# EspressoSystems/Push-CDN

Measured on NVIDIA H100. Metric: broadcast fan-out egress GB/s (1 KiB x 2^20 subscribers per GPU, 1 topic); msgs/s and % of HBM peak alongside, higher is better.
Workload: dtype u8

## Files before the change

### push-cdn_b200/csrc/engine.cu

```cuda
#include "engine_internal.h"

namespace pcdn_detail {
thread_local std::string g_err;
int fail(int code, const std::string& msg) { g_err = msg; return code; }
}

namespace {

int flush_journal(pcdn_engine* e) {
  HostTables& t = *e->tables;
  if (!e->has_device) { t.clear_dirty(); return 0; }
  const Geometry& g = e->geo;
  bool any = !t.dirty_sub.empty() || !t.dirty_brk.empty() || !t.dirty_owner.empty() || !t.dirty_slots.empty() ||
             !t.dirty_keys.empty();
  if (!any) return 0;
  const uint32_t Ws = e->shard_W(), W = g.W;
  const bool full_keys = t.dirty_keys.size() > (size_t)g.max_keys / 16 + 64;
  const bool full_sub = t.dirty_sub.size() > t.sub.size() / 16 + 64;
  const bool full_slots = t.dirty_slots.size() > t.cuckoo.size() / 16 + 64;
  e->h_slot.clear(); e->h_kslot.clear(); e->h_kbytes.clear();
  if (!full_slots) for (uint32_t i : t.dirty_slots) e->h_slot.push_back(UpdSlot{i, t.cuckoo[i]});
  if (!full_keys) for (uint32_t k : t.dirty_keys) {
    e->h_kslot.push_back(k);
    size_t at = e->h_kbytes.size();
// ... 148 lines not shown
  if (sh.dev.pool && !fused) s.spans_mapped = false;
  s.w.spans = s.spans_mapped ? s.d_spans_map : s.d_spans_dev;
  s.w.overflow = s.spans_mapped ? s.d_ovf_map : s.d_ovf_dev;
  const bool zero_in_kernel = fused && !devparse && !retry;
  const bool zero_in_match = !fused && !devparse && !retry && !has_direct && s.in.n_bcast > 0;
  if (s.timed) CUDA_TRY(cudaEventRecord(s.ev[0], st));
  if (retry) {
    launch_pool_retry_begin(sh.dev, s.w, st);
  } else {
    if (!zero_in_kernel && !zero_in_match) launch_batch_begin(sh.dev, s.w, s.in, has_direct, st);
    if (devparse) launch_parse(sh.dev, s.w, s.in, st);
    if (has_direct && !fused) launch_direct(sh.dev, s.w, s.in, n_direct, st);
  }
  if (s.timed) CUDA_TRY(cudaEventRecord(s.ev[1], st));
  if (fused) {
    launch_ctrl_small(sh.dev, s.w, s.in, has_direct, hs.targeted, zero_in_kernel, s.d_stats_pub, retry, st);
    if (s.timed) { CUDA_TRY(cudaEventRecord(s.ev[2], st)); CUDA_TRY(cudaEventRecord(s.ev[3], st)); }
  } else {
    if (!retry) launch_match(sh.dev, s.w, s.in, zero_in_match ? s.w.stats : nullptr, hs.targeted, st);
    if (s.timed) CUDA_TRY(cudaEventRecord(s.ev[2], st));
    if (!retry) launch_plan(sh.dev, s.w, s.in, st);
    launch_offsets(sh.dev, s.w, s.in, has_direct, sh.n_sms, st);
    if (s.timed) CUDA_TRY(cudaEventRecord(s.ev[3], st));
  }
  if (!s.spans_mapped) {
    CUDA_TRY(cudaEventRecord(s.ev_ctrl, st));
    CUDA_TRY(cudaStreamWaitEvent(cs, s.ev_ctrl, 0));
    CUDA_TRY(cudaMemcpyAsync(s.h_early, s.w.stats, sizeof(BatchStats), cudaMemcpyDeviceToHost, cs));
    CUDA_TRY(cudaEventRecord(s.ev_early, cs));
    if (ps != st) CUDA_TRY(cudaStreamWaitEvent(ps, s.ev_ctrl, 0));
  }
  if (s.timed) CUDA_TRY(cudaEventRecord(s.ev[4], ps));
  uint32_t pack_variant = e->cfg.pack_variant;
  if (!((pack_variant >> 8) & 15u)) pack_variant |= (fat_overlap ? 3u : 4u) << 8;
  const bool has_ref = e->cfg.ref_min_bytes && (hs.device_input || hs.max_raw_len >= e->cfg.ref_min_bytes);
  const bool published = launch_pack(sh.dev, s.w, s.in, n_direct, pack_variant, sh.n_sms, has_ref, fused ? nullptr : s.d_stats_pub, ps);
  if (s.timed) CUDA_TRY(cudaEventRecord(s.ev[5], ps));
// ... 577 lines not shown
    DEV_ALLOC(d.pool_state, 1);
    launch_pool_init(d, sh.stream);
  }
  CUDA_TRY(cudaMemsetAsync(d.sub, 0, (size_t)g.T * Ws * 4, sh.stream));
  CUDA_TRY(cudaMemsetAsync(d.brk, 0, (size_t)Ws * 4, sh.stream));
  CUDA_TRY(cudaMemsetAsync(d.owner_conn, 0xFF, (size_t)g.max_owners * 4, sh.stream));
  CUDA_TRY(cudaMemsetAsync(d.cuckoo, 0, (size_t)g.nbuckets * 4 * sizeof(CuckooEntry), sh.stream));
  CUDA_TRY(cudaMemsetAsync(d.keys, 0, (size_t)g.max_keys * g.key_stride, sh.stream));
  CUDA_TRY(cudaMemsetAsync(d.ptail, 0, (size_t)Ns * 4, sh.stream));
  CUDA_TRY(cudaMemsetAsync(d.used, 0, (size_t)Ns * 4, sh.stream));

  const uint32_t M = c.max_batch_msgs, MB = c.max_batch_bcast;
  const size_t cap_fat = (size_t)c.max_batch_deliveries;
  const size_t cap_thin = std::min<size_t>(c.max_batch_deliveries, (size_t)M * (kFatMin - 1));
  sh.slots.resize(c.batch_slots);
  for (ShardSlot& s : sh.slots) {
    DEV_ALLOC(s.d_arena, e->arena_cap);
    Work& w = s.w;
    DEV_ALLOC(w.B, (size_t)MB * Ws);
    DEV_ALLOC(w.wpre, (size_t)MB * Ws);
    DEV_ALLOC(w.cnt, (size_t)MB * d.nblk);
    DEV_ALLOC(w.base, (size_t)MB * d.nblk);
    DEV_ALLOC(w.done, MB);
    CUDA_TRY(cudaMemsetAsync(w.done, 0, (size_t)MB * 4, sh.stream));
    DEV_ALLOC(w.D, M);
    DEV_ALLOC(w.dconn, M);
    DEV_ALLOC(w.eb_fat, (size_t)M + 1);
    DEV_ALLOC(w.eb_thin, (size_t)M + 1);
    DEV_ALLOC(w.tbase, (size_t)M + 1);
    DEV_ALLOC(w.scan_tmp, 4 * ((size_t)M / 256 + 2));
    DEV_ALLOC(w.cls, M);
    DEV_ALLOC(w.cm_rank, (size_t)M + 1);
    DEV_ALLOC(w.cm_list, MB);
    DEV_ALLOC(w.jidx, M);
    DEV_ALLOC(w.efat, cap_fat);
    DEV_ALLOC(w.ecm, cap_fat);
    DEV_ALLOC(w.cmrun, std::min<size_t>(((size_t)MB + kCmGroup - 1) / kCmGroup * Ns, 2 * cap_fat + Ns));
    DEV_ALLOC(w.ethin, cap_thin);
    w.cap_fat = (uint32_t)std::min<size_t>(cap_fat, 0xFFFFFFFFu);
    w.cap_thin = (uint32_t)std::min<size_t>(cap_thin, 0xFFFFFFFFu);
    DEV_ALLOC(w.dcount, (size_t)Ns + 2);
    DEV_ALLOC(w.dloc, (size_t)Ns + 2);
    DEV_ALLOC(w.dtile, (size_t)Ns / 1024 + 3);
    DEV_ALLOC(w.dlist, M);
    DEV_ALLOC(w.hot_list, (size_t)M / kHotMin + 2);
    DEV_ALLOC(w.hot_bitmap, (size_t)kHotCtas * ((size_t)M / 32 + 1));
    DEV_ALLOC(w.scan_done, 1);
    CUDA_TRY(cudaMemsetAsync(w.scan_done, 0, 4, sh.stream));
    DEV_ALLOC(w.edir, M);
    DEV_ALLOC(w.dstart, (size_t)Ns + 1);
    DEV_ALLOC(w.dend, (size_t)Ns + 1);
    DEV_ALLOC(w.dstamp, (size_t)Ns + 1);
    CUDA_TRY(cudaMemsetAsync(w.dstamp, 0, ((size_t)Ns + 1) * 4, sh.stream));
    w.stamp = 0;
    DEV_ALLOC(w.batch_units, Ns);
    if (d.pool) {
      DEV_ALLOC(w.cbase, Ns);
      DEV_ALLOC(w.lb_state, (size_t)Ns / 256 + 1);
      DEV_ALLOC(w.lb_tot, (size_t)Ns / 256 + 1);
      CUDA_TRY(cudaMemsetAsync(w.lb_state, 0, ((size_t)Ns / 256 + 1) * 8, sh.stream));
    }
    w.pool_unblock = 0;
    const size_t span_entries = (size_t)2 * Ns * (d.span_runs ? 3 : 2) / 2;
    DEV_ALLOC(s.d_spans_dev, span_entries);
    DEV_ALLOC(s.d_ovf_dev, Ns);
    if (sh.direct_publish) {
      PIN_ALLOC_MAPPED(s.h_spans, s.d_spans_map, span_entries);
      PIN_ALLOC_MAPPED(s.h_overflow, s.d_ovf_map, (size_t)Ns);
    } else {
      PIN_ALLOC(s.h_spans, span_entries);
// ... 781 lines not shown
int pcdn_release_batch(pcdn_engine* e, uint64_t batch_id) {
  GUARD_BEGIN
  LOCK;
  const int si = find_slot_index(e, batch_id);
  if (si < 0) return fail(PCDN_ENOENT, "unknown batch id");
  if (e->inflight.empty() || e->inflight.front() != batch_id)
    return fail(PCDN_EINVAL, "batches must be released oldest first");
  Slot& s = e->slots[si];
  for (Shard& sh : e->shards) {
    DeviceGuard dg(sh.device);
    ShardSlot& ss = sh.slots[si];
    const bool payload_copy = s.device_input && e->delivers_by_ref();
    if (!ss.polled && (!s.device_input || payload_copy))
      CUDA_TRY(cudaEventSynchronize((e->sharded && !payload_copy) ? ss.ev_ingest : ss.ev_done));
    CUDA_TRY(cudaStreamWaitEvent(sh.stream, ss.ev_done, 0));
    launch_release(sh.dev, ss.w.batch_units, ss.w.stats, sh.stream);
    CUDA_TRY(cudaGetLastError());
  }
  e->inflight.erase(e->inflight.begin());
  s.state = SLOT_FREE;
  e->inflight_bytes -= std::min(e->inflight_bytes, s.ingress_bytes);
  s.ingress_bytes = 0;
  e->stats.released_batches++;
  {
    const double ms = std::chrono::duration<double, std::milli>(std::chrono::steady_clock::now() - s.t_launch).count();
    e->stats.latency_ms_sum += ms;
    const uint64_t us = (uint64_t)(ms * 1000.0);
    int bucket = 0;
    while (bucket < 15 && us >= (16ull << bucket)) bucket++;
    e->stats.latency_hist_us[bucket]++;
  }
// ... 115 lines not shown
```

### push-cdn_b200/csrc/engine_internal.h

```cpp
#pragma once
#include <cuda_runtime.h>

#include <algorithm>
#include <chrono>
#include <cstdio>
#include <cstring>
#include <memory>
#include <mutex>
#include <new>
#include <string>
#include <thread>
#include <vector>

#include "frame_parse.h"
#include "host_state.h"
#include "kernels.cuh"
#include "nccl_dl.h"
#include "pcdn_fanout.h"

using namespace pcdn;

namespace pcdn_detail {

int fail(int code, const std::string& msg);
// ... 69 lines not shown
struct Shard {
  int device = 0;
  uint32_t gindex = 0;
  int n_sms = 132;
  bool direct_publish = false;
  uint8_t* h_rings = nullptr;
  cudaStream_t stream = nullptr, pack_stream = nullptr, copy_stream = nullptr, ingest_stream = nullptr;
  bool own_stream = false;
  DevState dev{};
  std::vector<ShardSlot> slots;
  uint8_t* jstage_h = nullptr; uint8_t* jstage_d = nullptr; size_t jstage_cap = 0;
  cudaEvent_t ev_journal = nullptr; bool ev_journal_pending = false;
  std::vector<Upd32> h_u32;
  NcclComm comm = nullptr;
  int nccl_ranks = 0;
  int prev_slot[2] = {-1, -1};
  bool fat_only = false;
  cudaEvent_t ev_submit = nullptr;
  std::vector<void*> dev_allocs, pin_allocs;
};

struct Slot {
  int state = SLOT_FREE;
  uint64_t batch_id = 0;
  bool device_input = false;
  uint8_t* h_arena = nullptr;
  size_t arena_used = 0;
  std::vector<uint8_t> kind, flags;
  std::vector<uint32_t> slot_off16, raw_len, aux_off, aux_len, bcast_index;
  std::vector<uint16_t> topics;
// ... 119 lines not shown
```

### push-cdn_b200/csrc/kernels.cu

```cuda
#include "kernels.cuh"

#include <atomic>

#include "frame_parse_core.h"

namespace pcdn {

std::atomic<unsigned long long> g_kernel_launches{0};
#define PCDN_COUNT_LAUNCH (void)g_kernel_launches.fetch_add(1, std::memory_order_relaxed)

unsigned long long kernel_launches() { return g_kernel_launches.load(std::memory_order_relaxed); }
void count_kernel_launch() { PCDN_COUNT_LAUNCH; }

__device__ __forceinline__ uint32_t lane_id() { return threadIdx.x & 31; }

__device__ __forceinline__ uint32_t warp_incl_scan(uint32_t v) {
  const uint32_t lane = lane_id();
#pragma unroll
  for (int o = 1; o < 32; o <<= 1) {
    uint32_t n = __shfl_up_sync(0xffffffffu, v, o);
    if (lane >= (uint32_t)o) v += n;
  }
  return v;
}
// ... 288 lines not shown

void launch_batch_begin(const DevState&, const Work& w, const BatchIn&, bool, cudaStream_t st) {
  cudaMemsetAsync(w.stats, 0, sizeof(BatchStats), st);
}

void launch_direct(const DevState& s, const Work& w, const BatchIn& b, uint32_t n_direct, cudaStream_t st) {
  const uint32_t n = b.n_msgs;
  const uint32_t nseg = s.N + 1, ntiles = (nseg + 1023) / 1024;
  cudaMemsetAsync(w.dcount, 0, (size_t)(s.N + 2) * 4, st);
  PCDN_COUNT_LAUNCH, k_direct_lookup<<<(n * 8 + 255) / 256, 256, 0, st>>>(s, b, w);
  PCDN_COUNT_LAUNCH, k_dscan<<<ntiles, 256, 0, st>>>(w, nseg, ntiles);
  PCDN_COUNT_LAUNCH, k_dfill<<<(n + 255) / 256, 256, 0, st>>>(b, w);
  if (n_direct > kHotMin) PCDN_COUNT_LAUNCH, k_dsort_hot<<<kHotCtas, 256, 0, st>>>(b, w, (n + 31) / 32);
}


__device__ __forceinline__ bool msg_topic(const DevState& s, const BatchIn& b, uint32_t fl, uint32_t toff, uint32_t i, uint32_t* t) {
  if (fl & MSGF_TOPICS_U8) {
    const uint8_t* tb = b.arena + toff;
    if ((fl & MSGF_PRUNE) && !topic_kept(tb, i, s.n_valid_topics)) return false;
    *t = tb[i];
  } else {
    *t = b.topics[toff + i];
  }
  return *t < s.T;
}

__device__ uint32_t event_bit(const DevState& s, const BatchIn& b, uint32_t m, uint32_t wd, uint32_t k, uint32_t e0, uint32_t e1) {
  const uint32_t fl = b.flags[m], toff = b.aux_off[m], tn = b.aux_len[m];
  for (uint32_t i = 0; i < tn; i++) {
// ... 53 lines not shown
    for (uint32_t i = 0; i < tn; i++) {
      if ((fl & MSGF_PRUNE) && !topic_kept(tb, i, s.n_valid_topics)) continue;
      const uint32_t t = tb[i];
      if (t < s.T) word |= s.sub[(size_t)t * s.W + wd];
    }
  } else {
    for (uint32_t i = 0; i < tn; i++) {
      const uint32_t t = b.topics[toff + i];
      if (t < s.T) word |= s.sub[(size_t)t * s.W + wd];
    }
  }
  if (b.n_events) apply_events<1>(s, b, m, wd, &word);
  if (fl & MSGF_USERS_ONLY) word &= ~s.brk[wd];
  return word;
}
template <bool EVENTS, bool TARGET>
__global__ void __launch_bounds__(256) k_match(DevState s, BatchIn b, Work w, BatchStats* zero) {
  if (zero && blockIdx.x == 0 && blockIdx.y == 0 && threadIdx.x < sizeof(BatchStats) / 4) reinterpret_cast<uint32_t*>(zero)[threadIdx.x] = 0;
  const uint32_t j = blockIdx.y, lane = lane_id();
  const uint32_t blk = blockIdx.x * 8 + (threadIdx.x >> 5);
  if (blk >= s.nblk) return;
  const uint32_t m = b.bcast_index[j];
  const uint32_t w0 = blk * kBlockWords + lane * 8;
  const uint32_t toff = b.aux_off[m], tn = b.aux_len[m], fl = b.flags[m];
  uint4 lo = make_uint4(0, 0, 0, 0), hi = make_uint4(0, 0, 0, 0);
  auto or_row = [&](uint32_t t) {
    if (t >= s.T) return;
    const uint4* row = reinterpret_cast<const uint4*>(s.sub + (size_t)t * s.W + w0);
    const uint4 a = row[0], c = row[1];
    lo.x |= a.x; lo.y |= a.y; lo.z |= a.z; lo.w |= a.w;
    hi.x |= c.x; hi.y |= c.y; hi.z |= c.z; hi.w |= c.w;
  };
// ... 20 lines not shown
  if (TARGET && (fl & MSGF_TARGET)) {
    if (toff == kConnNone) {
      const uint4* br = reinterpret_cast<const uint4*>(s.brk + w0);
      lo = br[0]; hi = br[1];
    } else {
      const uint32_t local = toff - s.conn_base, bit = 1u << (local & 31u);
      const uint32_t q = local < s.N ? (local >> 5) - w0 : 8u;
      lo = make_uint4(q == 0 ? bit : 0u, q == 1 ? bit : 0u, q == 2 ? bit : 0u, q == 3 ? bit : 0u);
      hi = make_uint4(q == 4 ? bit : 0u, q == 5 ? bit : 0u, q == 6 ? bit : 0u, q == 7 ? bit : 0u);
    }
  }
  const uint32_t p0 = __popc(lo.x), p1 = p0 + __popc(lo.y), p2 = p1 + __popc(lo.z), p3 = p2 + __popc(lo.w);
  const uint32_t p4 = p3 + __popc(hi.x), p5 = p4 + __popc(hi.y), p6 = p5 + __popc(hi.z), p7 = p6 + __popc(hi.w);
  const uint32_t incl = warp_incl_scan(p7), ex = incl - p7;
  uint32_t last = 0;
  if (lane == 31) {
    w.cnt[(size_t)j * s.nblk + blk] = incl;
    __threadfence();
    last = atomicAdd(&w.done[j], 1u) == s.nblk - 1 ? 1u : 0u;
  }
  uint4* Bo = reinterpret_cast<uint4*>(w.B + (size_t)j * s.W + w0);
  Bo[0] = lo; Bo[1] = hi;
  uint4 pre;
  pre.x = ex | ((ex + p0) << 16); pre.y = (ex + p1) | ((ex + p2) << 16);
  pre.z = (ex + p3) | ((ex + p4) << 16); pre.w = (ex + p5) | ((ex + p6) << 16);
  *reinterpret_cast<uint4*>(w.wpre + (size_t)j * s.W + w0) = pre;
  if (__shfl_sync(0xffffffffu, last, 31)) {
    __threadfence();
    uint32_t carry = 0;
    for (uint32_t bb = 0; bb < s.nblk; bb += 32) {
      const uint32_t i = bb + lane;
      const uint32_t v = i < s.nblk ? __ldcg(w.cnt + (size_t)j * s.nblk + i) : 0;
      const uint32_t in = warp_incl_scan(v);
      if (i < s.nblk) w.base[(size_t)j * s.nblk + i] = carry + in - v;
      carry += __shfl_sync(0xffffffffu, in, 31);
    }
    if (lane == 0) { w.D[m] = carry; w.jidx[m] = j; w.done[j] = 0; }
  }
}
void launch_match(const DevState& s, const Work& w, const BatchIn& b, BatchStats* zero, bool targeted, cudaStream_t st) {
  if (!b.n_bcast) return;
  dim3 grid((s.nblk + 7) / 8, b.n_bcast);
  if (targeted) {
    if (b.n_events) PCDN_COUNT_LAUNCH, k_match<true, true><<<grid, 256, 0, st>>>(s, b, w, zero);
    else PCDN_COUNT_LAUNCH, k_match<false, true><<<grid, 256, 0, st>>>(s, b, w, zero);
  } else {
    if (b.n_events) PCDN_COUNT_LAUNCH, k_match<true, false><<<grid, 256, 0, st>>>(s, b, w, zero);
    else PCDN_COUNT_LAUNCH, k_match<false, false><<<grid, 256, 0, st>>>(s, b, w, zero);
  }
}

__device__ __forceinline__ uint32_t frame_vec_bytes(uint32_t raw_len) { return (4u + raw_len + 15u) & ~15u; }
__device__ __forceinline__ uint32_t frame_units(uint32_t raw_len) { return (4u + raw_len + kUnit - 1u) / kUnit; }
__device__ __forceinline__ bool by_ref(const DevState& s, uint32_t raw_len) { return raw_len >= s.ref_min; }
__device__ __forceinline__ uint32_t rec_units(const DevState& s, uint32_t raw_len) {
  return by_ref(s, raw_len) ? 1u : frame_units(raw_len);
}
__device__ __forceinline__ uint32_t tile_recipients(uint32_t frame_bytes) {
  const uint32_t chunk = min(frame_bytes, kChunkBytes);
  return max(32u, min(kTileRecipients, kFatTileBytes / chunk));
}

__device__ __forceinline__ void plan_classify(const DevState& s, const BatchIn& b, uint32_t m, uint32_t d, uint32_t* cls_out,
                                              uint32_t* tiles_out) {
  uint32_t cls = CLS_THIN, tiles = 0;
  if (d >= kFatMin) {
    const uint32_t len = b.raw_len[m];
    const bool ref = by_ref(s, len);
    const bool dense = !ref && ((uint64_t)d << kCmDenseShift) >= s.N && b.kind[m] == 4;
    if (dense && frame_units(len) * kUnit <= kCmMaxBytes) {
      cls = CLS_CM;
    } else {
      cls = CLS_FAT;
      const uint32_t nch = (frame_vec_bytes(len) + kChunkBytes - 1) / kChunkBytes;
      const uint32_t tr = tile_recipients(frame_vec_bytes(len));
      tiles = ref ? 0u : nch * ((d + tr - 1) / tr);
    }
  }
  *cls_out = cls; *tiles_out = tiles;
}

__global__ void __launch_bounds__(256) k_plan_a(DevState s, BatchIn b, Work w, uint32_t nblk) {
  __shared__ uint32_t sm[9];
  const uint32_t m = blockIdx.x * 256 + threadIdx.x;
  const bool valid = m < b.n_msgs;
  const uint32_t d = valid ? w.D[m] : 0;
  uint32_t cls, tiles;
  plan_classify(s, b, m, d, &cls, &tiles);
  uint32_t tot;
  uint32_t e0 = block256_excl_scan(cls != CLS_THIN ? d : 0, &tot, sm);
  if (threadIdx.x == 0) w.scan_tmp[blockIdx.x] = tot;
  uint32_t e1 = block256_excl_scan(cls == CLS_THIN ? d : 0, &tot, sm);
  if (threadIdx.x == 0) w.scan_tmp[nblk + blockIdx.x] = tot;
  uint32_t e2 = block256_excl_scan(tiles, &tot, sm);
  if (threadIdx.x == 0) w.scan_tmp[2 * nblk + blockIdx.x] = tot;
  uint32_t e3 = block256_excl_scan(cls == CLS_CM ? 1u : 0u, &tot, sm);
  if (threadIdx.x == 0) w.scan_tmp[3 * nblk + blockIdx.x] = tot;
  if (valid) { w.eb_fat[m] = e0; w.eb_thin[m] = e1; w.tbase[m] = e2; w.cm_rank[m] = e3; w.cls[m] = (uint8_t)cls; }
  if (gridDim.x == 1) {
    if (valid && cls == CLS_CM) w.cm_list[e3] = m;
    if (threadIdx.x == 0) {
      const uint32_t t0 = w.scan_tmp[0], t1 = w.scan_tmp[1], t2 = w.scan_tmp[2], t3 = w.scan_tmp[3];
      w.stats->n_fat_entries = t0; w.stats->n_thin_entries = t1; w.stats->n_fat_tiles = t2; w.stats->tile_cursor = 0;
      w.stats->n_cm = t3; w.stats->cm_cursor = 0;
      if (t0 > w.cap_fat || t1 > w.cap_thin) w.stats->status = 1;
      const uint32_t n = b.n_msgs;
      w.eb_fat[n] = t0; w.eb_thin[n] = t1; w.tbase[n] = t2; w.cm_rank[n] = t3;
    }
  }
}
__global__ void __launch_bounds__(256) k_plan_b(Work w, uint32_t nblk) {
  __shared__ uint32_t sm[9];
  const uint32_t q = blockIdx.x;
  uint32_t* t = w.scan_tmp + (size_t)q * nblk;
  uint32_t carry = 0;
  for (uint32_t bb = 0; bb < nblk; bb += 256) {
    const uint32_t i = bb + threadIdx.x;
    const uint32_t v = i < nblk ? t[i] : 0;
    uint32_t tot, ex = block256_excl_scan(v, &tot, sm);
    if (i < nblk) t[i] = ex + carry;
    carry += tot;
  }
  if (threadIdx.x == 0) {
    if (q == 0) { w.stats->n_fat_entries = carry; if (carry > w.cap_fat) w.stats->status = 1; }
// ... 7 lines not shown
  if (m < b.n_msgs) {
    w.eb_fat[m] += w.scan_tmp[blockIdx.x];
    w.eb_thin[m] += w.scan_tmp[nblk + blockIdx.x];
    w.tbase[m] += w.scan_tmp[2 * nblk + blockIdx.x];
    const uint32_t r = w.cm_rank[m] + w.scan_tmp[3 * nblk + blockIdx.x];
    w.cm_rank[m] = r;
    if (w.cls[m] == CLS_CM) w.cm_list[r] = m;
  } else if (m == b.n_msgs) {
    w.eb_fat[m] = w.stats->n_fat_entries;
    w.eb_thin[m] = w.stats->n_thin_entries;
    w.tbase[m] = w.stats->n_fat_tiles;
    w.cm_rank[m] = w.stats->n_cm;
  }
}
void launch_plan(const DevState& s, const Work& w, const BatchIn& b, cudaStream_t st) {
  if (b.n_bcast == 0) return;
  const uint32_t nblk = (b.n_msgs + 255) / 256;
  PCDN_COUNT_LAUNCH, k_plan_a<<<nblk, 256, 0, st>>>(s, b, w, nblk);
  if (nblk == 1) return;
  PCDN_COUNT_LAUNCH, k_plan_b<<<4, 256, 0, st>>>(w, nblk);
  PCDN_COUNT_LAUNCH, k_plan_c<<<(b.n_msgs + 1 + 255) / 256, 256, 0, st>>>(b, w, nblk);
}

struct ConnCursor {
  uint32_t pt, us, bu;
  uint32_t s1_off, s1_units, s1_rec, s2_units, s2_rec;
  uint32_t ovf, in2;
  uint32_t bytes;
};
__device__ __forceinline__ uint32_t alloc_record(ConnCursor& k, uint32_t u, uint32_t R, uint32_t raw_len) {
  if (k.ovf) return kOffInvalid;
  const bool wrap = k.pt + u > R;
  const uint32_t pad = wrap ? R - k.pt : 0, at = wrap ? 0 : k.pt;
  if (u > R || k.us + pad + u > R) { k.ovf = 1; return kOffInvalid; }
// ... 50 lines not shown
    if ((unsigned long long)p->head + total <= s.pool_units) ok = true;
    else if (total <= p->tail && p->used) { skip = s.pool_units - p->head; base = 0; ok = true; }
    else ok = false;
    if (p->used && p->head == p->tail) ok = false;
  } else {
    ok = p->head + total <= p->tail;
  }
  if (!ok) { bs->status = 2; p->blocked = 1; return; }
  p->head = base + total;
  p->used += total + skip;
  bs->pool_base = base; bs->pool_units = total; bs->pool_skip = skip;
}

template <bool HAS_DIRECT, int NT, bool SPARSE_BOUNDS, bool LOOKBACK>
__device__ __forceinline__ void offsets_body(const DevState& s, const BatchIn& b, const Work& w, uint32_t max_conns,
                                             uint32_t c, uint32_t vb, uint32_t nvb) {
  constexpr int NW = NT / 32;
  __shared__ uint32_t sm[NW + 1];
  __shared__ unsigned long long red[2][NW];
  __shared__ uint32_t span_base;
  if (w.stats->status) return;
  const uint32_t wd = c >> 5, lane = c & 31, lt = (1u << lane) - 1u;
  const uint32_t R = s.pool ? 0x7FFFFFFFu : s.ring_units;
  ConnCursor k;
  k.pt = s.pool ? 0u : s.ptail[c]; k.us = s.pool ? 0u : s.used[c]; k.bu = 0;
  k.s1_off = 0; k.s1_units = 0; k.s1_rec = 0; k.s2_units = 0; k.s2_rec = 0; k.ovf = 0; k.in2 = 0; k.bytes = 0;
  uint32_t dp = 0, de = 0;
  if (HAS_DIRECT) {
    if (SPARSE_BOUNDS) {
      if (w.dstamp[c] == w.stamp) { dp = w.dstart[c]; de = w.dend[c]; }
    } else {
      dp = dseg_start(w, c); de = dseg_start(w, c + 1);
      if (de - dp >= 2 && de - dp <= kHotMin) {
        for (uint32_t i = dp + 1; i < de; i++) {
          const uint32_t x = w.dlist[i];
          uint32_t j = i;
          while (j > dp && w.dlist[j - 1] > x) { w.dlist[j] = w.dlist[j - 1]; j--; }
          w.dlist[j] = x;
        }
      }
// ... 140 lines not shown
      uint32_t at = span_base + ex;
      if (k.s1_rec) runs[at++] = SpanRun{s.conn_base + c, run_len, s.pool ? k.s1_off : k.s1_off * kUnit, k.s1_units * kUnit, k.s1_rec, s.pool ? k.s1_units : 0u};
      if (k.s2_rec) runs[at] = SpanRun{s.conn_base + c, 1, 0, k.s2_units * kUnit, k.s2_rec, 0};
    }
  } else if (nsp) {
    uint32_t at = span_base + ex;
    if (k.s1_rec) w.spans[at++] = Span{s.conn_base + c, s.pool ? k.s1_off : k.s1_off * kUnit, k.s1_units * kUnit, k.s1_rec};
    if (k.s2_rec) w.spans[at] = Span{s.conn_base + c, 0, k.s2_units * kUnit, k.s2_rec};
  }
  if (k.ovf) {
    uint32_t i = atomicAdd(&w.stats->n_overflow, 1u);
    if (i < max_conns) w.overflow[i] = s.conn_base + c;
  }
}
template <bool HAS_DIRECT>
__global__ void __launch_bounds__(256) k_offsets(DevState s, BatchIn b, Work w, uint32_t max_conns) {
  offsets_body<HAS_DIRECT, 256, false, false>(s, b, w, max_conns, blockIdx.x * 256 + threadIdx.x, blockIdx.x, gridDim.x);
}
__global__ void __launch_bounds__(1024) k_pool_finish(DevState s, Work w, uint32_t nblk) {
  extern __shared__ uint32_t tb[];
  __shared__ uint32_t sm[33];
  __shared__ unsigned long long total_s;
  if (w.stats->status) return;
  unsigned long long carry = 0;
  for (uint32_t b0 = 0; b0 < nblk; b0 += 1024) {
    const uint32_t i = b0 + threadIdx.x;
    const uint32_t v = i < nblk ? w.lb_tot[i] : 0;
    uint32_t tot, ex = cta_excl_scan<32>(v, &tot, sm);
    const unsigned long long at = carry + ex;
    if (i < nblk) tb[i] = at > 0xFFFFFFFFull ? 0xFFFFFFFFu : (uint32_t)at;
    carry += tot;
  }
  if (threadIdx.x == 0) total_s = carry;
  __syncthreads();
  if (blockIdx.x == 0 && threadIdx.x == 0) pool_allocate(s, w, total_s);
  const uint32_t gt = blockIdx.x * 1024 + threadIdx.x, gn = gridDim.x * 1024;
  for (uint32_t c = gt; c < s.N; c += gn) w.cbase[c] += tb[c >> 8];
  if (s.span_runs) {
    SpanRun* r = reinterpret_cast<SpanRun*>(w.spans);
    const uint32_t n = w.stats->n_runs;
    for (uint32_t i = gt; i < n; i += gn) r[i].ring_off += tb[(r[i].conn0 - s.conn_base) >> 8];
  } else {
    const uint32_t n = w.stats->n_spans;
    for (uint32_t i = gt; i < n; i += gn) w.spans[i].ring_off += tb[(w.spans[i].conn - s.conn_base) >> 8];
  }
}

void launch_offsets(const DevState& s, const Work& w, const BatchIn& b, bool has_direct, int n_sms, cudaStream_t st) {
  if (has_direct) PCDN_COUNT_LAUNCH, k_offsets<true><<<s.N / 256, 256, 0, st>>>(s, b, w, s.N);
  else PCDN_COUNT_LAUNCH, k_offsets<false><<<s.N / 256, 256, 0, st>>>(s, b, w, s.N);
  if (s.pool) {
    const uint32_t nblk = s.N / 256;
    if (nblk * 4 > 48u * 1024) cudaFuncSetAttribute(k_pool_finish, cudaFuncAttributeMaxDynamicSharedMemorySize, (int)(nblk * 4));
    PCDN_COUNT_LAUNCH, k_pool_finish<<<std::min<uint32_t>((uint32_t)n_sms, (s.N + 8191) / 8192), 1024, nblk * 4, st>>>(s, w, nblk);
  }
}

__device__ __forceinline__ void cluster_sync_all() {
  asm volatile("barrier.cluster.arrive.release.aligned;\n\tbarrier.cluster.wait.acquire.aligned;" ::: "memory");
}
template <bool HAS_DIRECT, bool TARGET>
__global__ void __cluster_dims__(8, 1, 1) __launch_bounds__(1024, 1)
k_ctrl_small(DevState s, BatchIn b, Work w, int zero_stats, BatchStats* publish, int offsets_only) {
  __shared__ uint32_t sm[33];
  __shared__ uint32_t gbase[5];
  const uint32_t tid = threadIdx.x, rank = blockIdx.x;
  if (zero_stats && rank == 0 && tid < sizeof(BatchStats) / 4) reinterpret_cast<uint32_t*>(w.stats)[tid] = 0;

  if (HAS_DIRECT && rank == 0 && !offsets_only) {
    __shared__ uint32_t skey_s[kSmallCtrlMsgs], sorted_s[kSmallCtrlMsgs];
    __syncthreads();
    for (uint32_t g0 = 0; g0 < b.n_msgs * 8; g0 += 1024) direct_lookup_body<false>(s, b, w, g0 + tid);
    __syncthreads();
    const uint32_t n = b.n_msgs;
    if (tid < n) { const uint32_t t = w.dconn[tid]; skey_s[tid] = t == kConnNone ? s.N : t; }
    __syncthreads();
    if (tid < n) {
      const uint32_t key = skey_s[tid];
// ... 60 lines not shown
    if (valid) {
      w.eb_fat[m] = e0; w.eb_thin[m] = e1; w.tbase[m] = e2; w.cm_rank[m] = e3; w.cls[m] = (uint8_t)cls;
      if (cls == CLS_CM) w.cm_list[e3] = m;
    }
    if (tid == 0) {
      w.stats->n_fat_entries = t0; w.stats->n_thin_entries = t1; w.stats->n_fat_tiles = t2; w.stats->tile_cursor = 0;
      w.stats->n_cm = t3; w.stats->cm_cursor = 0;
      if (t0 > w.cap_fat || t1 > w.cap_thin) w.stats->status = 1;
      const uint32_t n = b.n_msgs;
      w.eb_fat[n] = t0; w.eb_thin[n] = t1; w.tbase[n] = t2; w.cm_rank[n] = t3;
    }
  }
  cluster_sync_all();

  for (uint32_t c0 = 0; c0 < s.N; c0 += 8192)
    offsets_body<HAS_DIRECT, 1024, true, true>(s, b, w, s.N, c0 + rank * 1024 + tid, c0 / 1024 + rank, s.N / 1024);

  if (publish) {
    cluster_sync_all();
    if (rank == 0 && tid < sizeof(BatchStats) / 4)
      reinterpret_cast<uint32_t*>(publish)[tid] = __ldcg(reinterpret_cast<const uint32_t*>(w.stats) + tid);
  }
}
void launch_ctrl_small(const DevState& s, const Work& w, const BatchIn& b, bool has_direct, bool targeted, bool zero_stats,
                       BatchStats* publish, bool offsets_only, cudaStream_t st) {
  const int z = zero_stats ? 1 : 0, oo = offsets_only ? 1 : 0;
  if (targeted) {
    if (has_direct) PCDN_COUNT_LAUNCH, k_ctrl_small<true, true><<<8, 1024, 0, st>>>(s, b, w, z, publish, oo);
    else PCDN_COUNT_LAUNCH, k_ctrl_small<false, true><<<8, 1024, 0, st>>>(s, b, w, z, publish, oo);
  } else {
    if (has_direct) PCDN_COUNT_LAUNCH, k_ctrl_small<true, false><<<8, 1024, 0, st>>>(s, b, w, z, publish, oo);
    else PCDN_COUNT_LAUNCH, k_ctrl_small<false, false><<<8, 1024, 0, st>>>(s, b, w, z, publish, oo);
  }
}

__global__ void k_pool_retry_begin(BatchStats* bs) {
  bs->status = 0;
  bs->n_deliveries = 0; bs->bytes_out = 0;
  bs->n_spans = 0; bs->n_runs = 0; bs->n_overflow = 0;
  bs->tile_cursor = 0; bs->cm_cursor = 0; bs->ctas_done = 0;
}
void launch_pool_retry_begin(const DevState& s, const Work& w, cudaStream_t st) {
  cudaMemsetAsync(w.lb_state, 0, ((size_t)s.N / 256 + 1) * 8, st);
  PCDN_COUNT_LAUNCH, k_pool_retry_begin<<<1, 1, 0, st>>>(w.stats);
}

__device__ __forceinline__ uint8_t* conn_out(const DevState& s, const Work& w, uint32_t conn, uint32_t pool_base) {
// ... 304 lines not shown
  }
  BatchStats* copy_publish = has_ref ? nullptr : publish;
  const bool direct_separate = n_direct >= kThinSeparateMin;
  const uint32_t ctas_per_sm = ((pack_variant >> 8) & 15u) ? ((pack_variant >> 8) & 15u) : 3;
  const uint32_t grid = (uint32_t)n_sms * ctas_per_sm;
  const int do_direct = (n_direct && !direct_separate) ? 1 : 0;
  if (b.n_bcast || do_direct)
    PCDN_COUNT_LAUNCH, k_pack<<<grid, 256, 0, st>>>(s, b, w, do_direct, direct_separate ? nullptr : copy_publish);
  const uint32_t dctas = ((pack_variant >> 12) & 15u) ? ((pack_variant >> 12) & 15u) : 8u;
  if (direct_separate) PCDN_COUNT_LAUNCH, k_pack_direct<<<(uint32_t)n_sms * dctas, 256, 0, st>>>(s, b, w, copy_publish);
  const bool launched = direct_separate || b.n_bcast || do_direct;
  if (has_ref && launched) PCDN_COUNT_LAUNCH, k_pack_ref<<<ref_ctas, 256, 0, st>>>(s, b, w, n_direct ? 1 : 0, publish);
  return launched;
}

__global__ void __launch_bounds__(256) k_release(DevState s, const uint32_t* __restrict__ batch_units,
                                                 const BatchStats* __restrict__ stats) {
  if (stats->status) return;
  const uint32_t i = blockIdx.x * blockDim.x + threadIdx.x;
  if (i * 4 < s.N) {
    const uint4 u = reinterpret_cast<const uint4*>(batch_units)[i];
    if (u.x | u.y | u.z | u.w) {
      uint4* p = reinterpret_cast<uint4*>(s.used) + i;
      uint4 v = *p;
      v.x -= u.x; v.y -= u.y; v.z -= u.z; v.w -= u.w;
      *p = v;
    }
  }
}
__global__ void k_pool_release(PoolState* p, const BatchStats* __restrict__ stats) {
  if (stats->status) return;
  p->used -= stats->pool_units + stats->pool_skip;
  p->tail = stats->pool_base + stats->pool_units;
  if (p->used == 0) { p->head = 0; p->tail = 0; }
}
__global__ void k_pool_init(PoolState* p) { p->head = 0; p->tail = 0; p->used = 0; p->blocked = 0; }
void launch_pool_init(const DevState& s, cudaStream_t st) {
  if (s.pool) PCDN_COUNT_LAUNCH, k_pool_init<<<1, 1, 0, st>>>(s.pool_state);
}
void launch_release(const DevState& s, const uint32_t* batch_units, const BatchStats* stats, cudaStream_t st) {
  if (s.pool) { PCDN_COUNT_LAUNCH, k_pool_release<<<1, 1, 0, st>>>(s.pool_state, stats); return; }
  PCDN_COUNT_LAUNCH, k_release<<<(s.N / 4 + 255) / 256, 256, 0, st>>>(s, batch_units, stats);
}

}
```

### push-cdn_b200/csrc/kernels.cuh

```cuda
#pragma once
#include <cuda_runtime.h>
#include <stdint.h>

#include "hash.h"

namespace pcdn {

constexpr uint32_t kUnit = 32;
constexpr uint32_t kOffInvalid = 0xFFFFFFFFu;
constexpr uint32_t kCmBroken = 0xFFFFFFF0u;
constexpr uint32_t kConnNone = 0xFFFFFFFFu;
constexpr uint32_t kFatMin = 32;
constexpr uint32_t kChunkBytes = 16384;
constexpr uint32_t kTileRecipients = 1024;
constexpr uint32_t kFatTileBytes = 131072;
constexpr uint32_t kBlockWords = 256;
constexpr uint32_t kCmGroup = 8;
constexpr uint32_t kCmMaxBytes = 4096;
constexpr uint32_t kSmallCtrlConns = 65536;
constexpr uint32_t kSmallCtrlMsgs = 256;
constexpr uint32_t kSmallCtrlItems = 256;
constexpr uint32_t kThinSeparateMin = 2048;
constexpr uint32_t kHotMin = 32;
constexpr uint32_t kHotCtas = 32;
// ... 117 lines not shown
  uint32_t* dend;
  uint32_t* dstamp;
  uint32_t stamp;
  uint32_t* cbase;
  unsigned long long* lb_state;
  uint32_t* lb_tot;
  uint32_t pool_unblock;
  unsigned long long batch_id;
  uint32_t* batch_units;
  Span* spans;
  uint32_t* overflow;
  int8_t* msg_status;
  BatchStats* stats;
};

struct Upd32 { uint32_t arr, idx, val; };
struct UpdSlot { uint32_t slot; CuckooEntry e; };

void launch_apply_updates(const DevState& s, const Upd32* u32, uint32_t n32, const UpdSlot* us,
                          uint32_t nslot, const uint32_t* key_slots, const uint8_t* key_bytes,
                          uint32_t nkeys, cudaStream_t st);
void launch_batch_begin(const DevState& s, const Work& w, const BatchIn& b, bool has_direct, cudaStream_t st);
void launch_parse(const DevState& s, const Work& w, const BatchIn& b, cudaStream_t st);
void launch_direct(const DevState& s, const Work& w, const BatchIn& b, uint32_t n_direct, cudaStream_t st);
void launch_match(const DevState& s, const Work& w, const BatchIn& b, BatchStats* zero, bool targeted, cudaStream_t st);
void launch_plan(const DevState& s, const Work& w, const BatchIn& b, cudaStream_t st);
void launch_offsets(const DevState& s, const Work& w, const BatchIn& b, bool has_direct, int n_sms, cudaStream_t st);
void launch_ctrl_small(const DevState& s, const Work& w, const BatchIn& b, bool has_direct, bool targeted, bool zero_stats,
                       BatchStats* publish, bool offsets_only, cudaStream_t st);
void launch_pool_retry_begin(const DevState& s, const Work& w, cudaStream_t st);
bool launch_pack(const DevState& s, const Work& w, const BatchIn& b, uint32_t n_direct, uint32_t pack_variant, int n_sms,
                 bool has_ref, BatchStats* publish, cudaStream_t st);
void launch_release(const DevState& s, const uint32_t* batch_units, const BatchStats* stats, cudaStream_t st);
void launch_pool_init(const DevState& s, cudaStream_t st);
unsigned long long kernel_launches();
void count_kernel_launch();

}
```

Measured before the change: 3034.

## Defer ring releases into offsets kernel and fold small-batch planning into match

Ring-unit releases for completed batches are no longer a separate kernel. A bitmask of pending slots is recorded, and the next offsets or ctrl kernel subtracts those slots' per-connection units from used before computing offsets. Separately, for batches of up to 256 messages, the last match block to finish (found via an atomic counter) does the plan scan inside k_match with warp scans, so k_plan_a is not launched. This cuts kernel launches per batch, at the cost of shared unit buffers per slot, extra loads in offsets, and subtler ordering invariants around status and error paths.

```diff
diff --git a/push-cdn_b200/csrc/engine.cu b/push-cdn_b200/csrc/engine.cu
--- a/push-cdn_b200/csrc/engine.cu
+++ b/push-cdn_b200/csrc/engine.cu
@@ -186,13 +186,15 @@
   }
   if (s.timed) CUDA_TRY(cudaEventRecord(s.ev[1], st));
   if (fused) {
-    launch_ctrl_small(sh.dev, s.w, s.in, has_direct, hs.targeted, zero_in_kernel, s.d_stats_pub, retry, st);
+    launch_ctrl_small(sh.dev, s.w, s.in, has_direct, hs.targeted, zero_in_kernel, s.d_stats_pub, retry, sh.pending_release, st);
+    sh.pending_release.mask = 0;
     if (s.timed) { CUDA_TRY(cudaEventRecord(s.ev[2], st)); CUDA_TRY(cudaEventRecord(s.ev[3], st)); }
   } else {
     if (!retry) launch_match(sh.dev, s.w, s.in, zero_in_match ? s.w.stats : nullptr, hs.targeted, st);
     if (s.timed) CUDA_TRY(cudaEventRecord(s.ev[2], st));
     if (!retry) launch_plan(sh.dev, s.w, s.in, st);
-    launch_offsets(sh.dev, s.w, s.in, has_direct, sh.n_sms, st);
+    launch_offsets(sh.dev, s.w, s.in, has_direct, sh.n_sms, sh.pending_release, st);
+    sh.pending_release.mask = 0;
     if (s.timed) CUDA_TRY(cudaEventRecord(s.ev[3], st));
   }
   if (!s.spans_mapped) {
@@ -800,6 +802,9 @@
   const size_t cap_fat = (size_t)c.max_batch_deliveries;
   const size_t cap_thin = std::min<size_t>(c.max_batch_deliveries, (size_t)M * (kFatMin - 1));
   sh.slots.resize(c.batch_slots);
+  uint32_t* units = nullptr;
+  DEV_ALLOC(units, (size_t)c.batch_slots * Ns);
+  sh.pending_release = PendingRelease{units, 0};
   for (ShardSlot& s : sh.slots) {
     DEV_ALLOC(s.d_arena, e->arena_cap);
     Work& w = s.w;
@@ -807,8 +812,8 @@
     DEV_ALLOC(w.wpre, (size_t)MB * Ws);
     DEV_ALLOC(w.cnt, (size_t)MB * d.nblk);
     DEV_ALLOC(w.base, (size_t)MB * d.nblk);
-    DEV_ALLOC(w.done, MB);
-    CUDA_TRY(cudaMemsetAsync(w.done, 0, (size_t)MB * 4, sh.stream));
+    DEV_ALLOC(w.done, (size_t)MB + 1);
+    CUDA_TRY(cudaMemsetAsync(w.done, 0, ((size_t)MB + 1) * 4, sh.stream));
     DEV_ALLOC(w.D, M);
     DEV_ALLOC(w.dconn, M);
     DEV_ALLOC(w.eb_fat, (size_t)M + 1);
@@ -839,7 +844,7 @@
     DEV_ALLOC(w.dstamp, (size_t)Ns + 1);
     CUDA_TRY(cudaMemsetAsync(w.dstamp, 0, ((size_t)Ns + 1) * 4, sh.stream));
     w.stamp = 0;
-    DEV_ALLOC(w.batch_units, Ns);
+    w.batch_units = units + (size_t)(&s - sh.slots.data()) * Ns;
     if (d.pool) {
       DEV_ALLOC(w.cbase, Ns);
       DEV_ALLOC(w.lb_state, (size_t)Ns / 256 + 1);
@@ -1651,7 +1656,8 @@
     if (!ss.polled && (!s.device_input || payload_copy))
       CUDA_TRY(cudaEventSynchronize((e->sharded && !payload_copy) ? ss.ev_ingest : ss.ev_done));
     CUDA_TRY(cudaStreamWaitEvent(sh.stream, ss.ev_done, 0));
-    launch_release(sh.dev, ss.w.batch_units, ss.w.stats, sh.stream);
+    if (!sh.dev.pool && (uint32_t)si < kMaxPendingRelease) sh.pending_release.mask |= 1u << si;
+    else launch_release(sh.dev, ss.w.batch_units, ss.w.stats, sh.stream);
     CUDA_TRY(cudaGetLastError());
   }
   e->inflight.erase(e->inflight.begin());
diff --git a/push-cdn_b200/csrc/engine_internal.h b/push-cdn_b200/csrc/engine_internal.h
--- a/push-cdn_b200/csrc/engine_internal.h
+++ b/push-cdn_b200/csrc/engine_internal.h
@@ -107,6 +107,7 @@
   std::vector<Upd32> h_u32;
   NcclComm comm = nullptr;
   int nccl_ranks = 0;
+  PendingRelease pending_release{};
   int prev_slot[2] = {-1, -1};
   bool fat_only = false;
   cudaEvent_t ev_submit = nullptr;
diff --git a/push-cdn_b200/csrc/kernels.cu b/push-cdn_b200/csrc/kernels.cu
--- a/push-cdn_b200/csrc/kernels.cu
+++ b/push-cdn_b200/csrc/kernels.cu
@@ -326,6 +326,36 @@
   if (n_direct > kHotMin) PCDN_COUNT_LAUNCH, k_dsort_hot<<<kHotCtas, 256, 0, st>>>(b, w, (n + 31) / 32);
 }
 
+__device__ __forceinline__ uint32_t frame_vec_bytes(uint32_t raw_len) { return (4u + raw_len + 15u) & ~15u; }
+__device__ __forceinline__ uint32_t frame_units(uint32_t raw_len) { return (4u + raw_len + kUnit - 1u) / kUnit; }
+__device__ __forceinline__ bool by_ref(const DevState& s, uint32_t raw_len) { return raw_len >= s.ref_min; }
+__device__ __forceinline__ uint32_t rec_units(const DevState& s, uint32_t raw_len) {
+  return by_ref(s, raw_len) ? 1u : frame_units(raw_len);
+}
+__device__ __forceinline__ uint32_t tile_recipients(uint32_t frame_bytes) {
+  const uint32_t chunk = min(frame_bytes, kChunkBytes);
+  return max(32u, min(kTileRecipients, kFatTileBytes / chunk));
+}
+
+__device__ __forceinline__ void plan_classify(const DevState& s, const BatchIn& b, uint32_t m, uint32_t d, uint32_t* cls_out,
+                                              uint32_t* tiles_out) {
+  uint32_t cls = CLS_THIN, tiles = 0;
+  if (d >= kFatMin) {
+    const uint32_t len = b.raw_len[m];
+    const bool ref = by_ref(s, len);
+    const bool dense = !ref && ((uint64_t)d << kCmDenseShift) >= s.N && b.kind[m] == 4;
+    if (dense && frame_units(len) * kUnit <= kCmMaxBytes) {
+      cls = CLS_CM;
+    } else {
+      cls = CLS_FAT;
+      const uint32_t nch = (frame_vec_bytes(len) + kChunkBytes - 1) / kChunkBytes;
+      const uint32_t tr = tile_recipients(frame_vec_bytes(len));
+      tiles = ref ? 0u : nch * ((d + tr - 1) / tr);
+    }
+  }
+  *cls_out = cls; *tiles_out = tiles;
+}
+
 
 __device__ __forceinline__ bool msg_topic(const DevState& s, const BatchIn& b, uint32_t fl, uint32_t toff, uint32_t i, uint32_t* t) {
   if (fl & MSGF_TOPICS_U8) {
@@ -409,8 +439,36 @@
   if (fl & MSGF_USERS_ONLY) word &= ~s.brk[wd];
   return word;
 }
+__device__ __forceinline__ void plan_in_match(const DevState& s, const BatchIn& b, const Work& w) {
+  const uint32_t lane = lane_id(), n = b.n_msgs;
+  uint32_t c0 = 0, c1 = 0, c2 = 0, c3 = 0;
+  for (uint32_t m0 = 0; m0 < n; m0 += 32) {
+    const uint32_t m = m0 + lane;
+    const bool valid = m < n;
+    const uint32_t d = valid ? __ldcg(w.D + m) : 0;
+    uint32_t cls, tiles;
+    plan_classify(s, b, m, d, &cls, &tiles);
+    const uint32_t v0 = cls != CLS_THIN ? d : 0, v1 = cls == CLS_THIN ? d : 0, v3 = cls == CLS_CM ? 1u : 0u;
+    const uint32_t i0 = warp_incl_scan(v0), i1 = warp_incl_scan(v1), i2 = warp_incl_scan(tiles), i3 = warp_incl_scan(v3);
+    if (valid) {
+      w.eb_fat[m] = c0 + i0 - v0; w.eb_thin[m] = c1 + i1 - v1; w.tbase[m] = c2 + i2 - tiles; w.cm_rank[m] = c3 + i3 - v3;
+      w.cls[m] = (uint8_t)cls;
+      if (cls == CLS_CM) w.cm_list[c3 + i3 - v3] = m;
+    }
+    c0 += __shfl_sync(0xffffffffu, i0, 31); c1 += __shfl_sync(0xffffffffu, i1, 31);
+    c2 += __shfl_sync(0xffffffffu, i2, 31); c3 += __shfl_sync(0xffffffffu, i3, 31);
+  }
+  if (lane == 0) {
+    w.stats->n_fat_entries = c0; w.stats->n_thin_entries = c1; w.stats->n_fat_tiles = c2; w.stats->tile_cursor = 0;
+    w.stats->n_cm = c3; w.stats->cm_cursor = 0;
+    if (c0 > w.cap_fat || c1 > w.cap_thin) w.stats->status = 1;
+    w.eb_fat[n] = c0; w.eb_thin[n] = c1; w.tbase[n] = c2; w.cm_rank[n] = c3;
+    w.done[b.n_bcast] = 0;
+  }
+}
+
 template <bool EVENTS, bool TARGET>
-__global__ void __launch_bounds__(256) k_match(DevState s, BatchIn b, Work w, BatchStats* zero) {
+__global__ void __launch_bounds__(256) k_match(DevState s, BatchIn b, Work w, BatchStats* zero, int plan) {
   if (zero && blockIdx.x == 0 && blockIdx.y == 0 && threadIdx.x < sizeof(BatchStats) / 4) reinterpret_cast<uint32_t*>(zero)[threadIdx.x] = 0;
   const uint32_t j = blockIdx.y, lane = lane_id();
   const uint32_t blk = blockIdx.x * 8 + (threadIdx.x >> 5);
@@ -461,6 +519,7 @@
   const uint32_t p4 = p3 + __popc(hi.x), p5 = p4 + __popc(hi.y), p6 = p5 + __popc(hi.z), p7 = p6 + __popc(hi.w);
   const uint32_t incl = warp_incl_scan(p7), ex = incl - p7;
   uint32_t last = 0;
+  __syncwarp();
   if (lane == 31) {
     w.cnt[(size_t)j * s.nblk + blk] = incl;
     __threadfence();
@@ -483,48 +542,24 @@
       carry += __shfl_sync(0xffffffffu, in, 31);
     }
     if (lane == 0) { w.D[m] = carry; w.jidx[m] = j; w.done[j] = 0; }
+    if (plan) {
+      uint32_t all = 0;
+      if (lane == 0) { __threadfence(); all = atomicAdd(&w.done[b.n_bcast], 1u) == b.n_bcast - 1 ? 1u : 0u; }
+      if (__shfl_sync(0xffffffffu, all, 0)) { __threadfence(); plan_in_match(s, b, w); }
+    }
   }
 }
 void launch_match(const DevState& s, const Work& w, const BatchIn& b, BatchStats* zero, bool targeted, cudaStream_t st) {
   if (!b.n_bcast) return;
   dim3 grid((s.nblk + 7) / 8, b.n_bcast);
+  const int plan = b.n_msgs <= 256 ? 1 : 0;
   if (targeted) {
-    if (b.n_events) PCDN_COUNT_LAUNCH, k_match<true, true><<<grid, 256, 0, st>>>(s, b, w, zero);
-    else PCDN_COUNT_LAUNCH, k_match<false, true><<<grid, 256, 0, st>>>(s, b, w, zero);
+    if (b.n_events) PCDN_COUNT_LAUNCH, k_match<true, true><<<grid, 256, 0, st>>>(s, b, w, zero, plan);
+    else PCDN_COUNT_LAUNCH, k_match<false, true><<<grid, 256, 0, st>>>(s, b, w, zero, plan);
   } else {
-    if (b.n_events) PCDN_COUNT_LAUNCH, k_match<true, false><<<grid, 256, 0, st>>>(s, b, w, zero);
-    else PCDN_COUNT_LAUNCH, k_match<false, false><<<grid, 256, 0, st>>>(s, b, w, zero);
-  }
-}
-
-__device__ __forceinline__ uint32_t frame_vec_bytes(uint32_t raw_len) { return (4u + raw_len + 15u) & ~15u; }
-__device__ __forceinline__ uint32_t frame_units(uint32_t raw_len) { return (4u + raw_len + kUnit - 1u) / kUnit; }
-__device__ __forceinline__ bool by_ref(const DevState& s, uint32_t raw_len) { return raw_len >= s.ref_min; }
-__device__ __forceinline__ uint32_t rec_units(const DevState& s, uint32_t raw_len) {
-  return by_ref(s, raw_len) ? 1u : frame_units(raw_len);
-}
-__device__ __forceinline__ uint32_t tile_recipients(uint32_t frame_bytes) {
-  const uint32_t chunk = min(frame_bytes, kChunkBytes);
-  return max(32u, min(kTileRecipients, kFatTileBytes / chunk));
-}
-
-__device__ __forceinline__ void plan_classify(const DevState& s, const BatchIn& b, uint32_t m, uint32_t d, uint32_t* cls_out,
-                                              uint32_t* tiles_out) {
-  uint32_t cls = CLS_THIN, tiles = 0;
-  if (d >= kFatMin) {
-    const uint32_t len = b.raw_len[m];
-    const bool ref = by_ref(s, len);
-    const bool dense = !ref && ((uint64_t)d << kCmDenseShift) >= s.N && b.kind[m] == 4;
-    if (dense && frame_units(len) * kUnit <= kCmMaxBytes) {
-      cls = CLS_CM;
-    } else {
-      cls = CLS_FAT;
-      const uint32_t nch = (frame_vec_bytes(len) + kChunkBytes - 1) / kChunkBytes;
-      const uint32_t tr = tile_recipients(frame_vec_bytes(len));
-      tiles = ref ? 0u : nch * ((d + tr - 1) / tr);
-    }
-  }
-  *cls_out = cls; *tiles_out = tiles;
+    if (b.n_events) PCDN_COUNT_LAUNCH, k_match<true, false><<<grid, 256, 0, st>>>(s, b, w, zero, plan);
+    else PCDN_COUNT_LAUNCH, k_match<false, false><<<grid, 256, 0, st>>>(s, b, w, zero, plan);
+  }
 }
 
 __global__ void __launch_bounds__(256) k_plan_a(DevState s, BatchIn b, Work w, uint32_t nblk) {
@@ -544,17 +579,6 @@
   uint32_t e3 = block256_excl_scan(cls == CLS_CM ? 1u : 0u, &tot, sm);
   if (threadIdx.x == 0) w.scan_tmp[3 * nblk + blockIdx.x] = tot;
   if (valid) { w.eb_fat[m] = e0; w.eb_thin[m] = e1; w.tbase[m] = e2; w.cm_rank[m] = e3; w.cls[m] = (uint8_t)cls; }
-  if (gridDim.x == 1) {
-    if (valid && cls == CLS_CM) w.cm_list[e3] = m;
-    if (threadIdx.x == 0) {
-      const uint32_t t0 = w.scan_tmp[0], t1 = w.scan_tmp[1], t2 = w.scan_tmp[2], t3 = w.scan_tmp[3];
-      w.stats->n_fat_entries = t0; w.stats->n_thin_entries = t1; w.stats->n_fat_tiles = t2; w.stats->tile_cursor = 0;
-      w.stats->n_cm = t3; w.stats->cm_cursor = 0;
-      if (t0 > w.cap_fat || t1 > w.cap_thin) w.stats->status = 1;
-      const uint32_t n = b.n_msgs;
-      w.eb_fat[n] = t0; w.eb_thin[n] = t1; w.tbase[n] = t2; w.cm_rank[n] = t3;
-    }
-  }
 }
 __global__ void __launch_bounds__(256) k_plan_b(Work w, uint32_t nblk) {
   __shared__ uint32_t sm[9];
@@ -592,10 +616,9 @@
   }
 }
 void launch_plan(const DevState& s, const Work& w, const BatchIn& b, cudaStream_t st) {
-  if (b.n_bcast == 0) return;
+  if (b.n_bcast == 0 || b.n_msgs <= 256) return;
   const uint32_t nblk = (b.n_msgs + 255) / 256;
   PCDN_COUNT_LAUNCH, k_plan_a<<<nblk, 256, 0, st>>>(s, b, w, nblk);
-  if (nblk == 1) return;
   PCDN_COUNT_LAUNCH, k_plan_b<<<4, 256, 0, st>>>(w, nblk);
   PCDN_COUNT_LAUNCH, k_plan_c<<<(b.n_msgs + 1 + 255) / 256, 256, 0, st>>>(b, w, nblk);
 }
@@ -676,16 +699,22 @@
 
 template <bool HAS_DIRECT, int NT, bool SPARSE_BOUNDS, bool LOOKBACK>
 __device__ __forceinline__ void offsets_body(const DevState& s, const BatchIn& b, const Work& w, uint32_t max_conns,
-                                             uint32_t c, uint32_t vb, uint32_t nvb) {
+                                             uint32_t c, uint32_t vb, uint32_t nvb, const PendingRelease& rel) {
   constexpr int NW = NT / 32;
   __shared__ uint32_t sm[NW + 1];
   __shared__ unsigned long long red[2][NW];
   __shared__ uint32_t span_base;
-  if (w.stats->status) return;
+  uint32_t us = s.pool ? 0u : s.used[c];
+  for (uint32_t m = rel.mask; m; m &= m - 1) us -= rel.units[(size_t)(__ffs(m) - 1) * s.N + c];
+  if (w.stats->status) {
+    if (rel.mask) s.used[c] = us;
+    w.batch_units[c] = 0;
+    return;
+  }
   const uint32_t wd = c >> 5, lane = c & 31, lt = (1u << lane) - 1u;
   const uint32_t R = s.pool ? 0x7FFFFFFFu : s.ring_units;
   ConnCursor k;
-  k.pt = s.pool ? 0u : s.ptail[c]; k.us = s.pool ? 0u : s.used[c]; k.bu = 0;
+  k.pt = s.pool ? 0u : s.ptail[c]; k.us = us; k.bu = 0;
   k.s1_off = 0; k.s1_units = 0; k.s1_rec = 0; k.s2_units = 0; k.s2_rec = 0; k.ovf = 0; k.in2 = 0; k.bytes = 0;
   uint32_t dp = 0, de = 0;
   if (HAS_DIRECT) {
@@ -856,8 +885,8 @@
   }
 }
 template <bool HAS_DIRECT>
-__global__ void __launch_bounds__(256) k_offsets(DevState s, BatchIn b, Work w, uint32_t max_conns) {
-  offsets_body<HAS_DIRECT, 256, false, false>(s, b, w, max_conns, blockIdx.x * 256 + threadIdx.x, blockIdx.x, gridDim.x);
+__global__ void __launch_bounds__(256) k_offsets(DevState s, BatchIn b, Work w, uint32_t max_conns, PendingRelease rel) {
+  offsets_body<HAS_DIRECT, 256, false, false>(s, b, w, max_conns, blockIdx.x * 256 + threadIdx.x, blockIdx.x, gridDim.x, rel);
 }
 __global__ void __launch_bounds__(1024) k_pool_finish(DevState s, Work w, uint32_t nblk) {
   extern __shared__ uint32_t tb[];
@@ -888,9 +917,10 @@
   }
 }
 
-void launch_offsets(const DevState& s, const Work& w, const BatchIn& b, bool has_direct, int n_sms, cudaStream_t st) {
-  if (has_direct) PCDN_COUNT_LAUNCH, k_offsets<true><<<s.N / 256, 256, 0, st>>>(s, b, w, s.N);
-  else PCDN_COUNT_LAUNCH, k_offsets<false><<<s.N / 256, 256, 0, st>>>(s, b, w, s.N);
+void launch_offsets(const DevState& s, const Work& w, const BatchIn& b, bool has_direct, int n_sms, const PendingRelease& rel,
+                    cudaStream_t st) {
+  if (has_direct) PCDN_COUNT_LAUNCH, k_offsets<true><<<s.N / 256, 256, 0, st>>>(s, b, w, s.N, rel);
+  else PCDN_COUNT_LAUNCH, k_offsets<false><<<s.N / 256, 256, 0, st>>>(s, b, w, s.N, rel);
   if (s.pool) {
     const uint32_t nblk = s.N / 256;
     if (nblk * 4 > 48u * 1024) cudaFuncSetAttribute(k_pool_finish, cudaFuncAttributeMaxDynamicSharedMemorySize, (int)(nblk * 4));
@@ -903,7 +933,7 @@
 }
 template <bool HAS_DIRECT, bool TARGET>
 __global__ void __cluster_dims__(8, 1, 1) __launch_bounds__(1024, 1)
-k_ctrl_small(DevState s, BatchIn b, Work w, int zero_stats, BatchStats* publish, int offsets_only) {
+k_ctrl_small(DevState s, BatchIn b, Work w, int zero_stats, BatchStats* publish, int offsets_only, PendingRelease rel) {
   __shared__ uint32_t sm[33];
   __shared__ uint32_t gbase[5];
   const uint32_t tid = threadIdx.x, rank = blockIdx.x;
@@ -994,7 +1024,7 @@
   cluster_sync_all();
 
   for (uint32_t c0 = 0; c0 < s.N; c0 += 8192)
-    offsets_body<HAS_DIRECT, 1024, true, true>(s, b, w, s.N, c0 + rank * 1024 + tid, c0 / 1024 + rank, s.N / 1024);
+    offsets_body<HAS_DIRECT, 1024, true, true>(s, b, w, s.N, c0 + rank * 1024 + tid, c0 / 1024 + rank, s.N / 1024, rel);
 
   if (publish) {
     cluster_sync_all();
@@ -1003,14 +1033,14 @@
   }
 }
 void launch_ctrl_small(const DevState& s, const Work& w, const BatchIn& b, bool has_direct, bool targeted, bool zero_stats,
-                       BatchStats* publish, bool offsets_only, cudaStream_t st) {
+                       BatchStats* publish, bool offsets_only, const PendingRelease& rel, cudaStream_t st) {
   const int z = zero_stats ? 1 : 0, oo = offsets_only ? 1 : 0;
   if (targeted) {
-    if (has_direct) PCDN_COUNT_LAUNCH, k_ctrl_small<true, true><<<8, 1024, 0, st>>>(s, b, w, z, publish, oo);
-    else PCDN_COUNT_LAUNCH, k_ctrl_small<false, true><<<8, 1024, 0, st>>>(s, b, w, z, publish, oo);
+    if (has_direct) PCDN_COUNT_LAUNCH, k_ctrl_small<true, true><<<8, 1024, 0, st>>>(s, b, w, z, publish, oo, rel);
+    else PCDN_COUNT_LAUNCH, k_ctrl_small<false, true><<<8, 1024, 0, st>>>(s, b, w, z, publish, oo, rel);
   } else {
-    if (has_direct) PCDN_COUNT_LAUNCH, k_ctrl_small<true, false><<<8, 1024, 0, st>>>(s, b, w, z, publish, oo);
-    else PCDN_COUNT_LAUNCH, k_ctrl_small<false, false><<<8, 1024, 0, st>>>(s, b, w, z, publish, oo);
+    if (has_direct) PCDN_COUNT_LAUNCH, k_ctrl_small<true, false><<<8, 1024, 0, st>>>(s, b, w, z, publish, oo, rel);
+    else PCDN_COUNT_LAUNCH, k_ctrl_small<false, false><<<8, 1024, 0, st>>>(s, b, w, z, publish, oo, rel);
   }
 }
 
@@ -1345,9 +1375,7 @@
   return launched;
 }
 
-__global__ void __launch_bounds__(256) k_release(DevState s, const uint32_t* __restrict__ batch_units,
-                                                 const BatchStats* __restrict__ stats) {
-  if (stats->status) return;
+__global__ void __launch_bounds__(256) k_release(DevState s, const uint32_t* __restrict__ batch_units) {
   const uint32_t i = blockIdx.x * blockDim.x + threadIdx.x;
   if (i * 4 < s.N) {
     const uint4 u = reinterpret_cast<const uint4*>(batch_units)[i];
@@ -1371,7 +1399,7 @@
 }
 void launch_release(const DevState& s, const uint32_t* batch_units, const BatchStats* stats, cudaStream_t st) {
   if (s.pool) { PCDN_COUNT_LAUNCH, k_pool_release<<<1, 1, 0, st>>>(s.pool_state, stats); return; }
-  PCDN_COUNT_LAUNCH, k_release<<<(s.N / 4 + 255) / 256, 256, 0, st>>>(s, batch_units, stats);
-}
-
-}
+  PCDN_COUNT_LAUNCH, k_release<<<(s.N / 4 + 255) / 256, 256, 0, st>>>(s, batch_units);
+}
+
+}
diff --git a/push-cdn_b200/csrc/kernels.cuh b/push-cdn_b200/csrc/kernels.cuh
--- a/push-cdn_b200/csrc/kernels.cuh
+++ b/push-cdn_b200/csrc/kernels.cuh
@@ -155,6 +155,12 @@
   BatchStats* stats;
 };
 
+constexpr uint32_t kMaxPendingRelease = 32;
+struct PendingRelease {
+  const uint32_t* units;
+  uint32_t mask;
+};
+
 struct Upd32 { uint32_t arr, idx, val; };
 struct UpdSlot { uint32_t slot; CuckooEntry e; };
 
@@ -166,9 +172,10 @@
 void launch_direct(const DevState& s, const Work& w, const BatchIn& b, uint32_t n_direct, cudaStream_t st);
 void launch_match(const DevState& s, const Work& w, const BatchIn& b, BatchStats* zero, bool targeted, cudaStream_t st);
 void launch_plan(const DevState& s, const Work& w, const BatchIn& b, cudaStream_t st);
-void launch_offsets(const DevState& s, const Work& w, const BatchIn& b, bool has_direct, int n_sms, cudaStream_t st);
+void launch_offsets(const DevState& s, const Work& w, const BatchIn& b, bool has_direct, int n_sms, const PendingRelease& rel,
+                    cudaStream_t st);
 void launch_ctrl_small(const DevState& s, const Work& w, const BatchIn& b, bool has_direct, bool targeted, bool zero_stats,
-                       BatchStats* publish, bool offsets_only, cudaStream_t st);
+                       BatchStats* publish, bool offsets_only, const PendingRelease& rel, cudaStream_t st);
 void launch_pool_retry_begin(const DevState& s, const Work& w, cudaStream_t st);
 bool launch_pack(const DevState& s, const Work& w, const BatchIn& b, uint32_t n_direct, uint32_t pack_variant, int n_sms,
                  bool has_ref, BatchStats* publish, cudaStream_t st);
```

New measurement: 3043 (median of 6 runs). About the same (+0.3%).
